# ypear/crdt

Measured on AMD Instinct MI355X. Metric: CRDT items merged/sec at 1/2/4/8 MI355X + % of HBM roofline, higher is better.
Workload: dtype u8/u32 (integer byte-stream + index work)

## Files before the change

### crdt_amd/csrc/yc_decode.hip

```cpp
#include <algorithm>
#include <cstdlib>

#include "yc_work.h"

namespace yc {

__device__ __forceinline__ uint64_t win8(const uint8_t* __restrict__ b, uint32_t p) {
  const uint32_t* d = (const uint32_t*)(b + (p & ~3u));
  return ((uint64_t)d[0] | ((uint64_t)d[1] << 32)) >> ((p & 3u) * 8);
}
__device__ __forceinline__ uint32_t win4(const uint8_t* __restrict__ b, uint32_t p) {
  const uint32_t* d = (const uint32_t*)(b + (p & ~3u));
  return __builtin_amdgcn_alignbyte(d[1], d[0], p & 3u);
}
struct RegWin {
  uint32_t r0, r1, r2, r3, r4, r5;
  uint32_t T;
  __device__ __forceinline__ static uint32_t sel(uint32_t m, uint32_t a1, uint32_t a0) { return (a1 & m) | (a0 & ~m); }
  __device__ __forceinline__ uint32_t word(uint32_t k) const {
    const uint32_t m0 = 0u - (k & 1u), m1 = 0u - ((k >> 1) & 1u), m2 = 0u - ((k >> 2) & 1u);
    const uint32_t a0 = sel(m0, r1, r0), a1 = sel(m0, r3, r2), a2 = sel(m0, r5, r4);
    return sel(m2, a2, sel(m1, a1, a0));
  }
  __device__ __forceinline__ uint32_t byte(uint32_t i) const { return (word(i >> 2) >> ((i & 3u) * 8)) & 0xFFu; }
// ... 2298 lines not shown
    uint32_t* out = k ? o1 : o0;
    uint32_t sum = 0;
    for (uint32_t i = a; i < e; ++i) sum += i < nwords ? (uint32_t)__popcll(bits[i]) : 0u;
    part[t] = sum;
    __syncthreads();
    for (uint32_t off = 1; off < COUNT_LANES; off <<= 1) {
      const uint32_t v = t >= off ? part[t - off] : 0u;
      __syncthreads();
      part[t] += v;
      __syncthreads();
    }
    uint32_t run = part[t] - sum;
    for (uint32_t i = a; i < e; ++i) { out[i] = run; run += i < nwords ? (uint32_t)__popcll(bits[i]) : 0u; }
    __syncthreads();
  }
}

void launch_struct_count(const Work& w, hipStream_t s) {
  const uint32_t nwords = (w.nbytes + 63) / 64;
  if (nwords + 1 <= COUNT_SMALL) {
    hipLaunchKernelGGL(k_count_small, dim3(1), dim3(COUNT_LANES), 0, s, w.final_bits, w.wcnt, w.sec_bits, w.wsec, nwords);
    return;
  }
  hipLaunchKernelGGL(k_popc, dim3(nwords / 256 + 1), dim3(256), 0, s, w.final_bits, w.scratch, nwords);
  scan_u32(w.tmp, w.tmp_bytes, w.scratch, w.wcnt, nwords + 1, s);
  hipLaunchKernelGGL(k_popc, dim3(nwords / 256 + 1), dim3(256), 0, s, w.sec_bits, w.scratch, nwords);
  scan_u32(w.tmp, w.tmp_bytes, w.scratch, w.wsec, nwords + 1, s);
}
void launch_struct_scatter(const Work& w, hipStream_t s) {
  const uint32_t nwords = (w.nbytes + 63) / 64;
  hipLaunchKernelGGL(k_scatter_pos, dim3(std::min<uint32_t>(nwords / 256 + 1, 4096)), dim3(256), 0, s, w.final_bits, w.wcnt, nwords, w.s_pos,
                     w.cap_structs, &w.ctr->err, w.nwin > 1 ? w.s_win : nullptr, w.win_shift);
}

void launch_section_clients(const Work& w, uint32_t nsections, hipStream_t s) {
  if (!nsections) return;
  hipLaunchKernelGGL(k_section_rank, dim3((nsections + 255) / 256), dim3(256), 0, s, w, nsections);
}

__device__ __forceinline__ uint32_t nth_lane(uint64_t x, uint32_t n) {
  for (uint32_t i = 0; i < n; ++i) x &= x - 1;
  return (uint32_t)__ffsll((long long)x) - 1;
}

__global__ __launch_bounds__(256) void k_ds_decode(Work w) {
  const uint32_t lane = threadIdx.x & 63;
// ... 812 lines not shown
__device__ __forceinline__ void struct_clock_at(const Work& w, uint32_t i, uint32_t nstructs, uint32_t states) {
  const uint32_t si = w.s_sec[i];
  const Section sec = w.sections[si];
  const uint64_t off = w.s_lenscan[i] - w.s_lenscan[sec.first_idx];
  const uint64_t clock = (uint64_t)sec.clock + off;
  const uint32_t len = w.s_len[i];
  const uint64_t endc = clock + len;
  if (endc > 0xFFFFFFFFull) { raise_err(&w.ctr->err, ERR_DECODE); return; }
  w.s_clock[i] = (uint32_t)clock;
  if (!states) return;
  const uint32_t ref = w.s_info[i] & 31u;
  if (ref == REF_SKIP) {
    atomicAdd(&w.ctr->items, (unsigned long long)len);
    return;
  }
  const bool last = i + 1 == nstructs || w.s_sec[i + 1] != si || (w.s_info[i + 1] & 31u) == REF_SKIP;
  if (last) atomicMax(&w.cl_state[w.s_cidx[i]], (uint32_t)endc);
}
__global__ void k_struct_clock(Work w, uint32_t nstructs, uint32_t states) {
  const uint32_t i = blockIdx.x * blockDim.x + threadIdx.x;
  if (i < nstructs) struct_clock_at(w, i, nstructs, states);
}

void launch_struct_decode(const Work& w, uint32_t nstructs, hipStream_t s) {
  if (!nstructs) return;
  hipLaunchKernelGGL(k_struct_decode, dim3((nstructs + 255) / 256), dim3(256), 0, s, w, nstructs);
  hipLaunchKernelGGL(k_struct_decode_deferred, dim3(std::min<uint32_t>(nstructs / 256 + 1, SD_DEFER_GRID)), dim3(256), 0, s, w);
}
void launch_struct_lenscan(const Work& w, uint32_t nstructs, hipStream_t s) {
  if (nstructs) scan_u32_to_u64(w.tmp, w.tmp_bytes, w.s_len, w.s_lenscan, nstructs + 1, s);
}

__device__ __forceinline__ void apply_caps_at(const Work& w, uint32_t c) {
  const uint32_t v = w.cl_vals[c];
  const uint32_t i = lower_bound_u32(w.cap_client, w.ncaps, v);
  const uint32_t cap = (i < w.ncaps && w.cap_client[i] == v) ? w.cap_clock[i] : 0u;
  if (ld_fresh(&w.cl_state[c]) > cap) w.cl_state[c] = cap;
}
__global__ void k_apply_caps(Work w) {
  const uint32_t c = blockIdx.x * blockDim.x + threadIdx.x;
  if (c < w.ctr->nclients) apply_caps_at(w, c);
}
__global__ void k_state_totals(Work w, uint32_t nstructs) {
  w.ctr->units = w.cl_base[w.ctr->nclients];
  w.ctr->in_len = w.s_lenscan[nstructs];
}
void launch_struct_clocks(const Work& w, uint32_t nstructs, hipStream_t s) {
  if (nstructs) hipLaunchKernelGGL(k_struct_clock, dim3((nstructs + 255) / 256), dim3(256), 0, s, w, nstructs, 0u);
}
void launch_states(const Work& w, uint32_t nstructs, uint32_t nsections, hipStream_t s) {
  if (nstructs) hipLaunchKernelGGL(k_struct_clock, dim3((nstructs + 255) / 256), dim3(256), 0, s, w, nstructs, 1u);
  if (w.capped && nsections) hipLaunchKernelGGL(k_apply_caps, dim3(nsections / 256 + 1), dim3(256), 0, s, w);
  scan_u32_to_u64(w.tmp, w.tmp_bytes, w.cl_state, w.cl_base, nsections + 1, s);
  hipLaunchKernelGGL(k_state_totals, dim3(1), dim3(1), 0, s, w, nstructs);
}

constexpr uint32_t DT_LANES = 256, DT_SMALL = 4096;
__global__ __launch_bounds__(DT_LANES) void k_decode_tail_small(Work w, uint32_t nstructs, uint32_t nsections) {
  __shared__ __attribute__((aligned(16))) uint32_t win[DT_LANES * SD_STRIDE];
  __shared__ uint64_t part[DT_LANES];
  const uint32_t t = threadIdx.x;
  if (nstructs == NONE) {
    if (w.ctr->err) return;
    nstructs = w.ctr->nstructs;
    nsections = w.ctr->nsections;
    if (nstructs > DT_SMALL || nsections + 1 > DT_LANES * 16) { if (t == 0) raise_err(&w.ctr->err, ERR_CAPACITY); return; }
  }
  if (w.dbg_bounds && (nstructs > w.cap_structs || nsections + 1 > w.cap_clients + 1)) {
    if (t == 0) bounds_fail(w.ctr, BOUNDS_DECODE_TAIL);
    return;
  }
  for (uint32_t i = t; i <= nsections; i += DT_LANES) { w.cl_start[i] = 0; w.cl_state[i] = 0; }
  for (uint32_t i = t; i < nstructs; i += DT_LANES) struct_decode_one<false>(w, i, win);
  __syncthreads();
  block_scan_u32_u64<DT_LANES>(w.s_len, w.s_lenscan, nstructs + 1, part);
  for (uint32_t i = t; i < nstructs; i += DT_LANES) struct_clock_at(w, i, nstructs, 1u);
  __syncthreads();
  const uint32_t nclients = w.ctr->nclients;
  if (w.capped) {
    for (uint32_t c = t; c < nclients; c += DT_LANES) apply_caps_at(w, c);
// ... 20 lines not shown
```

### crdt_amd/csrc/yc_engine.hip

```cpp
#include <cstddef>
#include <cstdio>
#include <cstring>
#include <string>
#include <vector>
#include <unordered_map>
#include <unordered_set>
#include <algorithm>
#include <memory>
#include <functional>

#include "yc_work.h"
#include "yc_host.h"
#include "yc_ingest.h"
#include "yc_comm.h"
#include "yc_sync.h"
#include "yc_json.h"
#include <thread>
#include <atomic>
#include "../../include/ycrdt.h"

using namespace yc;

namespace {

// ... 936 lines not shown
    uint32_t* fo = take<uint32_t>(V, B_FWCOFF, nu + 1, ok);
    if (ok) HIPCHK(hipMemcpyAsync(fo, b->fwc_off.data(), sizeof(uint32_t) * nu, hipMemcpyHostToDevice, e->stream));
    w.fwc_off = fo;
    if (!env_off("YCRDT_RTAB")) w.rtab = take<uint32_t>(V, B_RTAB, b->fwc_recs + 1, ok);
    if (w.rtab && !env_off("YCRDT_RANK_LAST")) w.rk = take<uint4>(V, B_RK, nu + 1, ok);
    const char* fw = getenv("YCRDT_FWC_WALK");
    w.fwc_walk = fw && atoi(fw) > 0 ? (uint32_t)atoi(fw) : 256u;
  }
  if (!ok) return fail(YCRDT_E_DEVICE, oom("decode workspace"));
  {
    size_t tb = prim_tmp_bytes(std::max<uint64_t>({B / 64 + 4, (uint64_t)nu + 2, (uint64_t)w.cap_sections + 2, 1024}),
                               (uint64_t)w.cap_sections + 2);
    w.tmp = take<uint8_t>(V, B_TMP, tb, ok);
    w.tmp_bytes = V[B_TMP].cap;
  }
  if (!ok) return fail(YCRDT_E_DEVICE, oom("scan scratch"));
  static_assert(sizeof(Counters) % 4 == 0, "counters are filled as words");
  fill_u32_multi({{(uint32_t*)w.ctr, sizeof(Counters) / 4, 0u},
                  {w.ufail, (uint64_t)nu + 1, 0u},
                  {w.usec_n, (uint64_t)nu + 1, 0u},
                  {(uint32_t*)w.final_bits, (uint64_t)nwords * 2, 0u},
                  {(uint32_t*)w.sec_bits, (uint64_t)nwords * 2, 0u}}, s);
  w.dbg_bounds = getenv("YCRDT_DEBUG_BOUNDS") && getenv("YCRDT_DEBUG_BOUNDS")[0] == '1' ? 1u : 0u;
  w.upre = b->pre_src >= 0 && !b->pre_check ? b->pre_u : NONE;
  if (w.upre != NONE) launch_predecoded(w, b->pre_u, b->pre, false, s);
  const bool dbg_yata = getenv("YCRDT_DEBUG_YATA") && getenv("YCRDT_DEBUG_YATA")[0] == '1';
  const bool dbg_dec = getenv("YCRDT_DEBUG_DECODE") && getenv("YCRDT_DEBUG_DECODE")[0] == '1';
  w.dbg = dbg_yata || dbg_dec ? take<unsigned long long>(V, B_DBG, 24, ok) : nullptr;
  if (w.dbg) HIPCHK(hipMemsetAsync(w.dbg, 0, 192, s));
  mark(e, "decode.direct");
  const bool split = sh && sh->comm && sh->nshards > 1 && !lazy;
  Work wd = w;
  if (split) {
    const int rc0 = split_decode_meta(e, b, sh, wd);
    if (rc0) return rc0;
  }
  const bool chunks = wd.ngroups || wd.nbig;
  if (chunks) {
    HIPCHK(hipEventRecord(e->side_fork, s));
    HIPCHK(hipStreamWaitEvent(e->side, e->side_fork, 0));
    launch_chunks(wd, e->side);
    HIPCHK(hipEventRecord(e->side_done, e->side));
  }
  launch_direct(wd, s);
  mark(e, "decode.chunk_wait");
  if (chunks) HIPCHK(hipStreamWaitEvent(s, e->side_done, 0));
// ... 25 lines not shown
  if (dbg_dec && w.dbg) {
    unsigned long long h[24];
    HIPCHK(hipMemcpy(h, w.dbg, sizeof(h), hipMemcpyDeviceToHost));
    fprintf(stderr, "[ycrdt decode] multi-section fast walk cycles: stage %llu walk %llu search %llu, walked structs %llu, sections vouched %llu\n",
            h[19], h[20], h[21], h[22], h[23]);
    fprintf(stderr, "[ycrdt decode] fastwalk: done %llu nsec %llu unsynced %llu | wave: done %llu unsettled %llu other %llu (chunk path: moved / jumped chunk entries) | k_spec exact parses %llu (%llu bytes) | multi-section left to k_walk, by reason 1-5: %llu %llu %llu %llu %llu (section %llu of %llu structs) | record mode: %llu sections evaluated by the walker, stopped at byte %llu of %llu\n",
            h[0], h[1], h[2], h[3], h[4], h[5], h[6], h[7], h[9], h[10], h[11], h[12], h[13], h[14], h[15], h[16], h[17], h[18]);
    HIPCHK(hipMemsetAsync(w.dbg, 0, 192, s));
  }
  if (rc == YCRDT_E_CAPACITY && !generous) return run_decode(e, b, lazy, D, true, sh);
  if (rc) return rc;
  const uint32_t nstructs = c.nstructs;
  const uint32_t nsections = c.nsections;
  w.cap_structs = nstructs + 64;
  w.cap_ds = c.ds_region + 64;
  w.cap_clients = nsections + 64;
  w.ds = lazy ? take<DsRange>(V, B_DS, w.cap_ds, ok) : nullptr;
  w.ds_tmp = take<DsRange>(V, B_DSTMP, w.cap_ds, ok);
  w.ds_len = nullptr;
  w.s_pos = take<uint32_t>(V, B_SPOS, w.cap_structs, ok);
  w.s_win = b->nwin > 1 ? take<uint8_t>(V, B_SWIN, w.cap_structs, ok) : nullptr;
  w.s_sec = take<uint32_t>(V, B_SSEC, w.cap_structs, ok);
  w.s_len = take<uint32_t>(V, B_SLEN, w.cap_structs + 1, ok);
  w.s_lenscan = take<uint64_t>(V, B_SLENSCAN, w.cap_structs + 1, ok);
  w.s_clock = take<uint32_t>(V, B_SCLOCK, w.cap_structs, ok);
  w.s_cidx = take<uint32_t>(V, B_SCIDX, w.cap_structs, ok);
  w.s_info = take<uint8_t>(V, B_SINFO, w.cap_structs, ok);
  w.s_ocidx = take<uint32_t>(V, B_SOC, w.cap_structs, ok);
  w.s_oclock = take<uint32_t>(V, B_SOK, w.cap_structs, ok);
  w.s_rcidx = take<uint32_t>(V, B_SRC, w.cap_structs, ok);
  w.s_rclock = take<uint32_t>(V, B_SRK, w.cap_structs, ok);
  w.s_pk = take<uint8_t>(V, B_SPK, w.cap_structs, ok);
  w.s_pa = take<uint32_t>(V, B_SPA, w.cap_structs, ok);
  w.s_pb = take<uint32_t>(V, B_SPB, w.cap_structs, ok);
  w.s_psub = take<uint32_t>(V, B_SPS, w.cap_structs, ok);
  w.s_psublen = take<uint32_t>(V, B_SPL, w.cap_structs, ok);
  w.s_cpos = take<uint32_t>(V, B_SCPOS, w.cap_structs, ok);
  w.s_cend = take<uint32_t>(V, B_SCEND, w.cap_structs, ok);
  w.s_celem = take<uint32_t>(V, B_SCELEM, w.cap_structs, ok);
  w.sd_defer = take<uint32_t>(V, B_SDDEFER, w.cap_structs, ok);
  w.cl_vals = take<uint32_t>(V, B_CLVALS, w.cap_clients + 1, ok);
  w.ch_key = nullptr;
  const uint32_t ch_slots = (uint32_t)next_pow2(std::max<uint64_t>(2ull * (nsections + 1), 64));
  uint64_t* ch_key = take<uint64_t>(V, B_CHKEY, ch_slots, ok);
  uint32_t* ch_val = take<uint32_t>(V, B_CHVAL, ch_slots, ok);
  w.cl_key = take<uint64_t>(V, B_CLKEY, w.cap_clients + 1, ok);
  w.cl_key2 = take<uint64_t>(V, B_CLKEY2, w.cap_clients + 1, ok);
// ... 52 lines not shown
    w.ch_key = ch_key;
    w.ch_val = ch_val;
    w.ch_mask = ch_slots - 1;
  } else if (nsections) {
    launch_client_table(w, nsections, s);
    fill_u32_multi({{(uint32_t*)ch_key, 2ull * ch_slots, 0xFFFFFFFFu}}, s);
    launch_client_hash(w, ch_key, ch_val, ch_slots - 1, s);
    w.ch_key = ch_key;
    w.ch_val = ch_val;
    w.ch_mask = ch_slots - 1;
  }
  mark(e, "decode.structs");
  if (quick) {
    launch_decode_tail_small(w, NONE, NONE, s);
    mark(e, "decode.clocks");
  } else if (!lazy && decode_tail_small(w, nstructs, nsections, s)) {
    mark(e, "decode.clocks");
  } else {
  launch_struct_decode(w, nstructs, s);
  mark(e, "decode.clocks");
  launch_struct_lenscan(w, nstructs, s);
  if (!lazy) {
    fill_u32_multi({{w.cl_start, (uint64_t)nsections + 1, 0u}, {w.cl_state, (uint64_t)nsections + 1, 0u}}, s);
    launch_states(w, nstructs, nsections, s);
  } else {
    HIPCHK(hipMemsetAsync(w.cl_start, 0, sizeof(uint32_t) * (nsections + 1), s));
    launch_struct_clocks(w, nstructs, s);
  }
  }
  HIPCHK(hipStreamWaitEvent(s, e->side_done, 0));
  rc = check(e, c, "struct decode");
  if (quick && rc == YCRDT_E_CAPACITY) return run_decode(e, b, lazy, D, true, sh);
  if (rc) return rc;
  const uint32_t nstructs_q = quick ? c.nstructs : nstructs, nsections_q = quick ? c.nsections : nsections;
  if (c.any_json) {
    w.jcap = std::max<uint32_t>(nstructs_q, 1);
    w.jlist = take<uint32_t>(V, B_JLIST, w.jcap, ok);
    if (!ok) return fail(YCRDT_E_DEVICE, oom("JSON list"));
    w.ntrusted = b->ntrusted;
    w.jskip_any = b->jpasses > 0 ? 1u : 0u;
    launch_json_structs(w, nstructs_q, s);
    rc = check(e, c, "JSON values");
    if (rc) return rc;
    if (c.njson) {
      bool restaged = false;
      if ((rc = json_rewrite(e, b, std::min(c.njson, w.jcap), sh, restaged))) return rc;
      if (restaged) return run_decode(e, b, lazy, D, generous, sh);
    }
  }
  D.noncanon = c.noncanon;
// ... 2664 lines not shown
```

### crdt_amd/csrc/yc_merge.hip

```cpp
#include <algorithm>
#include <cstdlib>

#include "yc_work.h"

namespace yc {



constexpr uint32_t LONG_UNITS = 32;
__device__ __forceinline__ uint64_t shfl64(uint64_t v, int l) {
  return ((uint64_t)(uint32_t)__shfl((uint32_t)(v >> 32), l) << 32) | (uint32_t)__shfl((uint32_t)v, l);
}
__device__ __forceinline__ void unit_owner(const Work& w, uint32_t nstructs, uint32_t s) {
  const uint32_t lane = threadIdx.x & 63;
  uint64_t gb = 0;
  uint32_t n = 0, fl = 0;
  if (s < nstructs) {
    const uint32_t ref = w.s_info[s] & 31u, cidx = w.s_cidx[s], clock = w.s_clock[s], len = w.s_len[s];
    const uint32_t st = w.cl_state[cidx];
    const uint64_t cb = w.cl_base[cidx];
    if (ref != REF_SKIP) {
      n = st > clock ? min(len, st - clock) : 0u;
      gb = cb + clock;
      fl = ref == REF_DELETED ? UF_DEL : (ref == REF_GC ? (UF_GC | UF_DEL) : 0u);
// ... 227 lines not shown
  if (blockIdx.x < nb) {
    const uint32_t s = blockIdx.x * blockDim.x + threadIdx.x;
    unit_owner(w, nstructs, s);
    unit_refs(w, nstructs, s);
  } else if (blockIdx.x < nb + nd) {
    unit_ds_apply(w, nclients, blockIdx.x - nb, BIG);
  } else if (BIG) {
    unit_ds_apply_big(w, nclients, blockIdx.x - nb - nd, nx);
  }
}
void launch_units_fill(const Work& w, uint64_t nunits, hipStream_t s) {
  fill_u32_multi({{w.u_owner, nunits, NONE}, {w.u_flags, nunits, 0u}}, s);
}
void launch_units(const Work& w, uint32_t nstructs, uint32_t nclients, uint32_t nds, uint64_t nunits, bool ds_big, hipStream_t s) {
  const uint32_t nb = (nstructs + 255) / 256, nd = nds && w.nupd ? (w.nupd + 3) / 4 : 0u;
  const uint32_t nx = nd && ds_big ? 256u : 0u;
  if (nb + nd) {
    if (nx) hipLaunchKernelGGL(k_units<true>, dim3(nb + nd + nx), dim3(256), 0, s, w, nstructs, nclients, nb, nd, nx);
    else hipLaunchKernelGGL(k_units<false>, dim3(nb + nd), dim3(256), 0, s, w, nstructs, nclients, nb, nd, 0u);
  }
  if (nx && w.ds_tails) hipLaunchKernelGGL(k_ds_tails, dim3(512), dim3(256), 0, s, w);
}

void launch_segments(const Work& w, uint32_t nclients, uint64_t nunits, hipStream_t s) {
  const uint32_t nwords = (uint32_t)((nunits + 63) / 64);
  if (nwords <= SEG_SMALL_WORDS) {
    hipLaunchKernelGGL(k_segments_small, dim3(1), dim3(SEG_LANES), 0, s, w, nunits);
    return;
  }
  hipLaunchKernelGGL(k_cuts, dim3(nwords / 4 + 1), dim3(256), 0, s, w, nunits);
  scan_u32(w.tmp, w.tmp_bytes, w.scratch, w.u_wpre, nwords + 1, s);
  hipLaunchKernelGGL(k_scatter_seg, dim3(nwords / 256 + 1), dim3(256), 0, s, w, nwords, nunits);
}

__device__ __forceinline__ uint64_t fnv_bytes(uint64_t h, const uint8_t* __restrict__ p, uint32_t n) {
  for (uint32_t i = 0; i < n; ++i) { h ^= p[i]; h *= 1099511628211ull; }
  return h;
}
__device__ __forceinline__ bool bytes_eq(const uint8_t* __restrict__ a, const uint8_t* __restrict__ b, uint32_t n) {
  for (uint32_t i = 0; i < n; ++i)
    if (a[i] != b[i]) return false;
  return true;
}
__device__ __forceinline__ bool same_list(const Work& w, uint32_t a, uint32_t b) {
  if (a == b) return true;
  const uint32_t pk = w.s_pk[a] & 3u;
  if (pk != (w.s_pk[b] & 3u)) return false;
  if (pk == 1) {
    const uint32_t n = w.s_pb[a];
    if (n != w.s_pb[b]) return false;
// ... 527 lines not shown
```

### crdt_amd/csrc/yc_prims.hip

```cpp
#include <algorithm>
#include <cstring>
#include <cstdlib>
#include <mutex>
#include <unordered_map>
#include <rocprim/rocprim.hpp>
#include "yc_work.h"

namespace yc {

struct SegMax64 {
  __host__ __device__ uint64_t operator()(uint64_t a, uint64_t b) const {
    return (a >> 32) == (b >> 32) ? (a > b ? a : b) : b;
  }
};

__global__ void k_fill_multi(FillBatch b) {
  const FillDesc d = b.d[blockIdx.y];
  for (uint64_t i = (uint64_t)blockIdx.x * blockDim.x + threadIdx.x; i < d.n; i += (uint64_t)gridDim.x * blockDim.x)
    d.p[i] = d.v;
}

void fill_u32_multi(std::initializer_list<FillDesc> fills, hipStream_t s) {
  FillBatch b{};
  uint64_t nmax = 0;
// ... 165 lines not shown
bool lb_launch(uint64_t tiles, uint32_t chains, hipStream_t s, LbChains& out) {
  std::lock_guard<std::mutex> g(lb_mu);
  LbState* st = lb_state(tiles * chains, s);
  if (!st) return false;
  out.state = st->state;
  out.stride = tiles;
  out.epoch = st->epoch;
  out.ord = st->state + st->tiles;
  out.ord_base = st->issued;
  st->issued += tiles;
  return true;
}

bool ordered_ids(uint64_t nblocks, hipStream_t s, OrderedIds& out) {
  std::lock_guard<std::mutex> g(lb_mu);
  LbState* st = lb_state(1, s);
  if (!st) return false;
  out.ctr = st->state + st->tiles;
  out.base = st->issued;
  st->issued += nblocks;
  return true;
}

void scan_u32(void* tmp, size_t tmpb, const uint32_t* in, uint32_t* out, uint64_t n, hipStream_t s) {
  if (!n) return;
  if (n <= SMALL_SCAN_MAX) {
    hipLaunchKernelGGL(k_scan_small<uint32_t>, dim3(1), dim3(SMALL_SCAN_LANES), 0, s, in, out, (uint32_t)n);
    return;
  }
  if (!getenv_flag("YCRDT_ROCPRIM_SCAN") && scan_lb<uint32_t>(in, out, n, s)) return;
  rocprim::exclusive_scan(tmp, tmpb, in, out, 0u, (size_t)n, rocprim::plus<uint32_t>(), s);
}

void scan_u32_to_u64(void* tmp, size_t tmpb, const uint32_t* in, uint64_t* out, uint64_t n, hipStream_t s) {
  if (!n) return;
  if (n <= SMALL_SCAN_MAX) {
    hipLaunchKernelGGL(k_scan_small<uint64_t>, dim3(1), dim3(SMALL_SCAN_LANES), 0, s, in, out, (uint32_t)n);
    return;
  }
  if (!getenv_flag("YCRDT_ROCPRIM_SCAN") && scan_lb<uint64_t>(in, out, n, s)) return;
  rocprim::exclusive_scan(tmp, tmpb, in, out, (uint64_t)0, (size_t)n, rocprim::plus<uint64_t>(), s);
}

void sort_u32(void* tmp, size_t tmpb, const uint32_t* in, uint32_t* out, uint64_t n, hipStream_t s) {
  if (!n) return;
  rocprim::radix_sort_keys(tmp, tmpb, in, out, (size_t)n, 0, 32, s);
// ... 35 lines not shown
```

### crdt_amd/csrc/yc_work.h

```cpp
#pragma once
#include <initializer_list>
#include "yc_common.h"
#include "yc_view.h"

namespace yc {

struct Counters {
  uint32_t err;
  uint32_t err_info;
  uint32_t nsections;
  uint32_t xchunks;
  uint32_t nds;
  uint32_t ndsclients;
  uint32_t nstructs;
  uint32_t nclients;
  uint32_t nunits_lo;
  uint32_t nunits_hi;
  uint32_t nsegs;
  uint32_t nout;
  uint32_t changed;
  uint32_t out_bytes;
  uint32_t sv_bytes;
  uint32_t nkeys;
  uint32_t nruns;
// ... 2 lines not shown
  uint32_t any_rorigin;
  uint32_t ds_big;
  uint32_t nsd_defer;
  uint32_t any_json;
  uint32_t narray_roots;
  uint32_t tgroups;
  uint32_t tbig;
  uint32_t ds_region;
  uint32_t nested;
  uint32_t nroots_sh[NSHARD];
  uint32_t nroots;
  uint32_t pad[12];
  uint32_t climb_open[40];
  uint32_t sync_changed[8];
  uint32_t noncanon;
  uint32_t lz_blocks;
  uint32_t njson;
  uint32_t ds_ntails;
  unsigned long long out_total;
  unsigned long long ds_base;
  unsigned long long items;
  unsigned long long units;
  unsigned long long in_len;
};

struct DsRange {
  uint32_t client;
  uint32_t clock;
  uint32_t len;
  uint32_t upd;
};

constexpr uint32_t WIN_SHIFT = 32;
__host__ __device__ inline uint64_t win_use(uint32_t shift) {
  return (1ull << shift) - (shift >= 28 ? (1ull << 20) : (1ull << 12));
}

struct Work {
  const uint8_t* bytes = nullptr;
  uint64_t nbytes = 0;
  uint32_t nwin = 1;
  uint32_t win_shift = WIN_SHIFT;
  const uint32_t* uwin = nullptr;
  const uint32_t* uoff = nullptr;
  const uint32_t* ulen = nullptr;
  const uint32_t* ugroup = nullptr;
  uint32_t nupd = 0;
  const uint32_t* udoc = nullptr;
  uint32_t ndocs = 1;
  const uint32_t* ulist = nullptr;
  uint32_t nbig = 0, nsmall = 0;
  uint32_t small_max = 0;
  uint32_t* fwsec = nullptr;
  uint4* fwc = nullptr;
  const uint32_t* fwc_off = nullptr;
  uint32_t* rtab = nullptr;
  uint4* rk = nullptr;
  uint32_t dbg_bounds = 0;
  uint32_t fwc_walk = 256;
  uint16_t* wlen = nullptr;
  uint32_t schunk = SCHUNK;
  uint32_t force_xtab = 0;
  uint32_t fwm_max = 0;
  uint32_t spec_hint = 2;
  uint32_t lazy = 0;
  unsigned long long* dbg = nullptr;
  const Group* groups = nullptr;
  uint32_t ngroups = 0;
  uint32_t cap_structs = 0, cap_sections = 0, cap_ds = 0, cap_dsclients = 0;
  uint64_t cap_units = 0;
  Counters* ctr = nullptr;
  uint64_t* spec_bits = nullptr;
  uint32_t* cexit = nullptr;
  uint32_t* sexit = nullptr;
  uint32_t* sent = nullptr;
  uint32_t* xtab = nullptr;
  uint32_t* tentry = nullptr;
  uint32_t* xlist = nullptr;
  uint32_t* ccnt = nullptr;
  uint32_t* coff = nullptr;
// ... 207 lines not shown
__device__ __forceinline__ uint32_t gidx() { return xcd_block() * blockDim.x + threadIdx.x; }

struct OrderedIds {
  unsigned long long* ctr = nullptr;
  unsigned long long base = 0;
};
bool ordered_ids(uint64_t nblocks, hipStream_t s, OrderedIds& out);
__device__ __forceinline__ uint32_t ordered_block_id(unsigned long long* ctr, unsigned long long base) {
  __shared__ uint32_t id;
  if (threadIdx.x == 0) id = (uint32_t)(atomicAdd(ctr, 1ull) - base);
  __syncthreads();
  return id;
}

constexpr uint64_t LB_VAL = (1ull << 40) - 1;
struct LbChains {
  unsigned long long* state = nullptr;
  uint64_t stride = 0;
  uint32_t epoch = 0;
  unsigned long long* ord = nullptr;
  unsigned long long ord_base = 0;
};
bool lb_launch(uint64_t tiles, uint32_t chains, hipStream_t s, LbChains& out);
__device__ __forceinline__ uint64_t lb_wave_lookback(unsigned long long* __restrict__ state, uint32_t tile, uint32_t epoch, uint64_t agg) {
  const uint32_t lane = threadIdx.x & 63;
  const unsigned long long ep = (unsigned long long)epoch << 42;
  if (tile == 0) {
    if (lane == 0) __hip_atomic_store(&state[0], ep | (2ull << 40) | (agg & LB_VAL), __ATOMIC_RELAXED, __HIP_MEMORY_SCOPE_AGENT);
    return 0;
  }
  if (lane == 0) __hip_atomic_store(&state[tile], ep | (1ull << 40) | (agg & LB_VAL), __ATOMIC_RELAXED, __HIP_MEMORY_SCOPE_AGENT);
  uint64_t pre = 0;
  for (int64_t j = (int64_t)tile - 1;; j -= 64) {
    const int64_t me = j - (int64_t)lane;
    uint32_t st = 2;
    uint64_t val = 0;
    if (me >= 0) {
      unsigned long long x;
      while (((x = __hip_atomic_load(&state[me], __ATOMIC_RELAXED, __HIP_MEMORY_SCOPE_AGENT)) >> 42) != epoch)
        __builtin_amdgcn_s_sleep(1);
      st = (uint32_t)(x >> 40) & 3u;
      val = x & LB_VAL;
    }
    const uint64_t done = __ballot(st == 2);
    const uint32_t stop = (uint32_t)__ffsll((long long)done) - 1;
    uint64_t part = lane <= stop ? val : 0ull;
    for (uint32_t off = 32; off > 0; off >>= 1) part += __shfl_xor(part, off);
    pre += part;
    if (done) break;
  }
  if (lane == 0) __hip_atomic_store(&state[tile], ep | (2ull << 40) | ((pre + agg) & LB_VAL), __ATOMIC_RELAXED, __HIP_MEMORY_SCOPE_AGENT);
  return pre;
}

__device__ __forceinline__ uint64_t client_hash(uint64_t k) {
  k ^= k >> 30; k *= 0xBF58476D1CE4E5B9ull;
  k ^= k >> 27; k *= 0x94D049BB133111EBull;
  return k ^ (k >> 31);
}
__device__ __forceinline__ uint32_t find_client(const Work& w, uint32_t nclients, uint32_t doc, uint32_t client) {
  if (w.ch_key) {
    const uint64_t key = w.udoc ? (((uint64_t)doc << 32) | client) : (uint64_t)client;
    for (uint32_t slot = (uint32_t)client_hash(key) & w.ch_mask;; slot = (slot + 1) & w.ch_mask) {
      const uint64_t k = w.ch_key[slot];
      if (k == key) return w.ch_val[slot];
      if (k == ~0ull) return NONE;
    }
  }
  if (!w.udoc) {
    const uint32_t i = lower_bound_u32(w.cl_vals, nclients, client);
    return (i < nclients && w.cl_vals[i] == client) ? i : NONE;
  }
  const uint64_t key = ((uint64_t)doc << 32) | client;
  uint32_t lo = 0, hi = nclients;
// ... 205 lines not shown
  uint32_t* order = nullptr;
  ViewSeg* segs = nullptr;
};
void launch_view(const Work& w, const ViewBufs& v, uint32_t nsegs, uint32_t nlists, uint32_t narr, hipStream_t s);

constexpr uint32_t UF_PRE = 6;
constexpr uint32_t UF_WALKED = 7;
struct PreMarks {
  uint64_t* fbits = nullptr;
  uint64_t* sbits = nullptr;
  Section* secs = nullptr;
  uint32_t* meta = nullptr;
  uint32_t nw = 0, cap_secs = 0;
};
void launch_state_marks(const Work& w, uint32_t nout, uint32_t nclients, const PreMarks& m, hipStream_t s);
void launch_predecoded(const Work& w, uint32_t u, const PreMarks& m, bool check, hipStream_t s);

void launch_chunks(const Work& w, hipStream_t s);
void launch_direct(const Work& w, hipStream_t s);
bool wave_decode(const Work& w);
void launch_client_hash(const Work& w, uint64_t* key, uint32_t* val, uint32_t mask, hipStream_t s);
bool sections_small(const Work& w, uint32_t nsections, uint64_t* key, uint32_t* val, uint32_t mask, hipStream_t s);
void launch_struct_count(const Work& w, hipStream_t s);
void launch_struct_scatter(const Work& w, hipStream_t s);
void launch_ds_bound(const Work& w, hipStream_t s);
bool count_ds_small(const Work& w, hipStream_t s);
void launch_ds_decode(const Work& w, hipStream_t s);
void launch_section_clients(const Work& w, uint32_t nsections, hipStream_t s);
void launch_client_table(Work& w, uint32_t nsections, hipStream_t s);
void launch_struct_decode(const Work& w, uint32_t nstructs, hipStream_t s);
void launch_struct_lenscan(const Work& w, uint32_t nstructs, hipStream_t s);
bool decode_tail_small(const Work& w, uint32_t nstructs, uint32_t nsections, hipStream_t s);
void launch_decode_tail_small(const Work& w, uint32_t nstructs, uint32_t nsections, hipStream_t s);
void launch_json_structs(const Work& w, uint32_t nstructs, hipStream_t s);
struct JItem {
  unsigned long long cpos;
  uint32_t clen;
  uint32_t len;
  uint32_t res;
  uint32_t pad;
};
void launch_json_canon(const Work& w, const uint32_t* list, uint32_t n, JItem* items, uint32_t* arena, uint32_t acap,
                       uint32_t lanes, const unsigned long long* offs, uint8_t* out, hipStream_t s);
void launch_states(const Work& w, uint32_t nstructs, uint32_t nsections, hipStream_t s);
void launch_struct_clocks(const Work& w, uint32_t nstructs, hipStream_t s);

void launch_units_fill(const Work& w, uint64_t nunits, hipStream_t s);
void launch_units(const Work& w, uint32_t nstructs, uint32_t nclients, uint32_t nds, uint64_t nunits, bool ds_big, hipStream_t s);
constexpr uint32_t DSA_WAVE = 4096;
void launch_segments(const Work& w, uint32_t nclients, uint64_t nunits, hipStream_t s);
void launch_segment_props_fill(const Work& w, uint32_t nsegs, hipStream_t s);
void launch_segment_props(const Work& w, uint32_t nsegs, uint32_t nclients, uint64_t nunits, hipStream_t s);
uint32_t run_key_resolution(const Work& w, uint32_t nsegs, hipStream_t s);
uint32_t run_descent(const Work& w, uint32_t nsegs, hipStream_t s, bool fold_overwrite);
void launch_mapx_flip(const Work& w, uint32_t nsegs, hipStream_t s);
void launch_mapx_fix(const Work& w, uint32_t nsegs, hipStream_t s);
bool merge_small_fits(uint64_t nsegs_bound);
void launch_merge_small(const Work& w, uint32_t nsegs, uint64_t nunits, hipStream_t s);
bool launch_merge_flags(const Work& w, uint32_t nsegs, hipStream_t s, bool fold_overwrite);
bool encode_runs_small(uint32_t nsegs);
void launch_merge_flags_only(const Work& w, uint32_t nsegs, hipStream_t s, bool fold_overwrite);
void launch_merge_tail(const Work& w, uint32_t nsegs, hipStream_t s);
void launch_key_shards(const Work& w, uint32_t nsegs, uint32_t nshards, uint32_t* key_shard, uint8_t* owner, hipStream_t s);
void launch_shard_mask(const Work& w, uint32_t nsegs, const uint8_t* owner, uint32_t shard, hipStream_t s);
void launch_shard_export(const Work& w, uint32_t nsegs, const uint8_t* owner, uint32_t shard, uint32_t* acc, hipStream_t s);
void launch_merge_final(const Work& w, uint32_t nsegs, hipStream_t s);
void run_dead_keys(const Work& w, uint32_t nsegs, hipStream_t s);
constexpr uint32_t DS_TAIL_MIN = 4096, DS_TAILS_CAP = 1u << 16;
// ... 49 lines not shown
```

Baseline: 3.864 billion.

## Fuse popcount scans, struct clocks, and segment cuts into single-pass look-back kernels

After: 4.036 billion, median of 6. +4.5%, better.

```diff
diff --git a/crdt_amd/csrc/yc_decode.hip b/crdt_amd/csrc/yc_decode.hip
--- a/crdt_amd/csrc/yc_decode.hip
+++ b/crdt_amd/csrc/yc_decode.hip
@@ -2344,6 +2344,7 @@
     hipLaunchKernelGGL(k_count_small, dim3(1), dim3(COUNT_LANES), 0, s, w.final_bits, w.wcnt, w.sec_bits, w.wsec, nwords);
     return;
   }
+  if (w.scan_fused && popc_scan2(w.final_bits, w.wcnt, w.sec_bits, w.wsec, nwords, s)) return;
   hipLaunchKernelGGL(k_popc, dim3(nwords / 256 + 1), dim3(256), 0, s, w.final_bits, w.scratch, nwords);
   scan_u32(w.tmp, w.tmp_bytes, w.scratch, w.wcnt, nwords + 1, s);
   hipLaunchKernelGGL(k_popc, dim3(nwords / 256 + 1), dim3(256), 0, s, w.sec_bits, w.scratch, nwords);
@@ -3202,13 +3203,134 @@
   if (i < nstructs) struct_clock_at(w, i, nstructs, states);
 }
 
+constexpr uint32_t SC_ITEMS = 16, SC_TILE = 256 * SC_ITEMS;
+constexpr uint64_t SC_SAT = 1ull << 33;
+__global__ __launch_bounds__(256) void k_struct_clock_lb(Work w, uint32_t nstructs, uint32_t states, uint32_t vec, LbChains lb) {
+  __shared__ uint64_t wsum[4], wlen[4];
+  __shared__ uint32_t whead[4];
+  __shared__ uint64_t tile_pre;
+  const uint32_t tile = ordered_block_id(lb.ord, lb.ord_base);
+  const uint32_t t = threadIdx.x, lane = t & 63, wv = t >> 6;
+  const uint64_t base = (uint64_t)tile * SC_TILE + (uint64_t)t * SC_ITEMS;
+  const bool full = vec && base + SC_ITEMS <= nstructs;
+  uint32_t sec[SC_ITEMS + 1], len[SC_ITEMS];
+  uint32_t info[SC_ITEMS + 1];
+  if (full) {
+#pragma unroll
+    for (uint32_t k = 0; k < SC_ITEMS / 4; ++k) {
+      const uint4 a = ((const uint4*)(w.s_sec + base))[k], b = ((const uint4*)(w.s_len + base))[k];
+      sec[4 * k] = a.x; sec[4 * k + 1] = a.y; sec[4 * k + 2] = a.z; sec[4 * k + 3] = a.w;
+      len[4 * k] = b.x; len[4 * k + 1] = b.y; len[4 * k + 2] = b.z; len[4 * k + 3] = b.w;
+    }
+    const uint4 q = *(const uint4*)(w.s_info + base);
+    const uint32_t qq[4] = {q.x, q.y, q.z, q.w};
+#pragma unroll
+    for (uint32_t k = 0; k < SC_ITEMS; ++k) info[k] = (qq[k >> 2] >> (8 * (k & 3))) & 0xFFu;
+  } else {
+#pragma unroll
+    for (uint32_t k = 0; k < SC_ITEMS; ++k) {
+      const bool in = base + k < nstructs;
+      sec[k] = in ? w.s_sec[base + k] : NONE;
+      len[k] = in ? w.s_len[base + k] : 0u;
+      info[k] = in ? (uint32_t)w.s_info[base + k] : 0u;
+    }
+  }
+  const bool nxt = base + SC_ITEMS < nstructs;
+  sec[SC_ITEMS] = nxt ? w.s_sec[base + SC_ITEMS] : NONE;
+  info[SC_ITEMS] = nxt ? (uint32_t)w.s_info[base + SC_ITEMS] : 0u;
+  const uint32_t psec = base > 0 && base <= nstructs ? w.s_sec[base - 1] : NONE;
+  uint64_t e[SC_ITEMS];
+  uint64_t run = 0, lsum = 0;
+  uint32_t heads = 0;
+#pragma unroll
+  for (uint32_t k = 0; k < SC_ITEMS; ++k) {
+    const bool in = base + k < nstructs;
+    const bool head = in && (base + k == 0 || sec[k] != (k ? sec[k - 1] : psec));
+    if (head) { run = w.sections[sec[k]].clock; heads |= 1u << k; }
+    run += len[k];
+    lsum += len[k];
+    e[k] = run;
+  }
+  uint64_t v = run;
+  uint32_t f = heads ? 1u : 0u;
+  for (uint32_t off = 1; off < 64; off <<= 1) {
+    const uint64_t pv = __shfl_up(v, off);
+    const uint32_t pf = __shfl_up(f, off);
+    if (lane >= off) { if (!f) v += pv; f |= pf; }
+  }
+  uint64_t ls = lsum;
+  for (uint32_t off = 32; off > 0; off >>= 1) ls += __shfl_xor(ls, off);
+  if (lane == 63) { wsum[wv] = v; whead[wv] = f; }
+  if (lane == 0) wlen[wv] = ls;
+  uint64_t cv = __shfl_up(v, 1);
+  uint32_t cf = __shfl_up(f, 1);
+  if (lane == 0) { cv = 0; cf = 0; }
+  __syncthreads();
+  uint64_t tv = 0;
+  uint32_t tf = 0;
+#pragma unroll
+  for (uint32_t x = 0; x < 4; ++x) {
+    if (x == wv) {
+      if (!cf) cv += tv;
+      cf |= tf;
+    }
+    if (whead[x]) { tv = wsum[x]; tf = 1u; } else tv += wsum[x];
+  }
+  if (wv == 0) {
+    const uint64_t pre = lb_wave_lookback(lb.state, tile, lb.epoch, tv, tf != 0, SC_SAT);
+    if (lane == 0) {
+      tile_pre = pre < SC_SAT ? pre : SC_SAT;
+      if (states) atomicAdd(&w.ctr->in_len_sh[tile & (NSHARD - 1)], (unsigned long long)(wlen[0] + wlen[1] + wlen[2] + wlen[3]));
+    }
+  }
+  __syncthreads();
+  const uint64_t carry = cf ? cv : cv + tile_pre;
+  const uint32_t first = heads ? (uint32_t)__ffs((int)heads) - 1 : SC_ITEMS;
+  uint32_t clk[SC_ITEMS];
+  uint32_t bad = 0;
+#pragma unroll
+  for (uint32_t k = 0; k < SC_ITEMS; ++k) {
+    const uint64_t endc = e[k] + (k < first ? carry : 0ull);
+    const bool in = base + k < nstructs;
+    const bool over = in && endc > 0xFFFFFFFFull;
+    bad |= (over ? 1u : 0u) << k;
+    clk[k] = (uint32_t)(endc - len[k]);
+    if (!in || over || !states) continue;
+    const uint32_t ref = info[k] & 31u;
+    if (ref == REF_SKIP) {
+      atomicAdd(&w.ctr->items, (unsigned long long)len[k]);
+      continue;
+    }
+    const bool last = base + k + 1 == nstructs || sec[k + 1] != sec[k] || (info[k + 1] & 31u) == REF_SKIP;
+    if (last) atomicMax(&w.cl_state[w.s_cidx[base + k]], (uint32_t)endc);
+  }
+  if (bad) raise_err(&w.ctr->err, ERR_DECODE);
+  if (full && !bad) {
+#pragma unroll
+    for (uint32_t k = 0; k < SC_ITEMS / 4; ++k)
+      ((uint4*)(w.s_clock + base))[k] = make_uint4(clk[4 * k], clk[4 * k + 1], clk[4 * k + 2], clk[4 * k + 3]);
+  } else {
+#pragma unroll
+    for (uint32_t k = 0; k < SC_ITEMS; ++k)
+      if (base + k < nstructs && !((bad >> k) & 1u)) w.s_clock[base + k] = clk[k];
+  }
+}
+static bool launch_struct_clock_lb(const Work& w, uint32_t nstructs, uint32_t states, hipStream_t s) {
+  const uint64_t tiles = ((uint64_t)nstructs + SC_TILE - 1) / SC_TILE;
+  LbChains lb;
+  if (!lb_launch(tiles, 1, s, lb)) return false;
+  const uint32_t vec = (((uintptr_t)w.s_sec | (uintptr_t)w.s_len | (uintptr_t)w.s_clock | (uintptr_t)w.s_info) & 15u) == 0;
+  hipLaunchKernelGGL(k_struct_clock_lb, dim3((uint32_t)tiles), dim3(256), 0, s, w, nstructs, states, vec, lb);
+  return true;
+}
+
 void launch_struct_decode(const Work& w, uint32_t nstructs, hipStream_t s) {
   if (!nstructs) return;
   hipLaunchKernelGGL(k_struct_decode, dim3((nstructs + 255) / 256), dim3(256), 0, s, w, nstructs);
   hipLaunchKernelGGL(k_struct_decode_deferred, dim3(std::min<uint32_t>(nstructs / 256 + 1, SD_DEFER_GRID)), dim3(256), 0, s, w);
 }
 void launch_struct_lenscan(const Work& w, uint32_t nstructs, hipStream_t s) {
-  if (nstructs) scan_u32_to_u64(w.tmp, w.tmp_bytes, w.s_len, w.s_lenscan, nstructs + 1, s);
+  if (nstructs && !clocks_fused(w, nstructs)) scan_u32_to_u64(w.tmp, w.tmp_bytes, w.s_len, w.s_lenscan, nstructs + 1, s);
 }
 
 __device__ __forceinline__ void apply_caps_at(const Work& w, uint32_t c) {
@@ -3221,21 +3343,29 @@
   const uint32_t c = blockIdx.x * blockDim.x + threadIdx.x;
   if (c < w.ctr->nclients) apply_caps_at(w, c);
 }
-__global__ void k_state_totals(Work w, uint32_t nstructs) {
+__global__ void k_state_totals(Work w, uint32_t nstructs, uint32_t fused) {
   w.ctr->units = w.cl_base[w.ctr->nclients];
-  w.ctr->in_len = w.s_lenscan[nstructs];
-}
-void launch_struct_clocks(const Work& w, uint32_t nstructs, hipStream_t s) {
+  if (!fused) { w.ctr->in_len = w.s_lenscan[nstructs]; return; }
+  unsigned long long n = 0;
+  for (uint32_t k = 0; k < NSHARD; ++k) n += w.ctr->in_len_sh[k];
+  w.ctr->in_len = n;
+}
+bool launch_struct_clocks(const Work& w, uint32_t nstructs, hipStream_t s) {
+  if (clocks_fused(w, nstructs)) return launch_struct_clock_lb(w, nstructs, 0u, s);
   if (nstructs) hipLaunchKernelGGL(k_struct_clock, dim3((nstructs + 255) / 256), dim3(256), 0, s, w, nstructs, 0u);
-}
-void launch_states(const Work& w, uint32_t nstructs, uint32_t nsections, hipStream_t s) {
-  if (nstructs) hipLaunchKernelGGL(k_struct_clock, dim3((nstructs + 255) / 256), dim3(256), 0, s, w, nstructs, 1u);
+  return true;
+}
+bool launch_states(const Work& w, uint32_t nstructs, uint32_t nsections, hipStream_t s) {
+  const bool fused = clocks_fused(w, nstructs);
+  if (fused) { if (!launch_struct_clock_lb(w, nstructs, 1u, s)) return false; }
+  else if (nstructs) hipLaunchKernelGGL(k_struct_clock, dim3((nstructs + 255) / 256), dim3(256), 0, s, w, nstructs, 1u);
   if (w.capped && nsections) hipLaunchKernelGGL(k_apply_caps, dim3(nsections / 256 + 1), dim3(256), 0, s, w);
   scan_u32_to_u64(w.tmp, w.tmp_bytes, w.cl_state, w.cl_base, nsections + 1, s);
-  hipLaunchKernelGGL(k_state_totals, dim3(1), dim3(1), 0, s, w, nstructs);
-}
-
-constexpr uint32_t DT_LANES = 256, DT_SMALL = 4096;
+  hipLaunchKernelGGL(k_state_totals, dim3(1), dim3(1), 0, s, w, nstructs, fused ? 1u : 0u);
+  return true;
+}
+
+constexpr uint32_t DT_LANES = 256;
 __global__ __launch_bounds__(DT_LANES) void k_decode_tail_small(Work w, uint32_t nstructs, uint32_t nsections) {
   __shared__ __attribute__((aligned(16))) uint32_t win[DT_LANES * SD_STRIDE];
   __shared__ uint64_t part[DT_LANES];
diff --git a/crdt_amd/csrc/yc_engine.hip b/crdt_amd/csrc/yc_engine.hip
--- a/crdt_amd/csrc/yc_engine.hip
+++ b/crdt_amd/csrc/yc_engine.hip
@@ -982,6 +982,7 @@
                   {(uint32_t*)w.final_bits, (uint64_t)nwords * 2, 0u},
                   {(uint32_t*)w.sec_bits, (uint64_t)nwords * 2, 0u}}, s);
   w.dbg_bounds = getenv("YCRDT_DEBUG_BOUNDS") && getenv("YCRDT_DEBUG_BOUNDS")[0] == '1' ? 1u : 0u;
+  w.scan_fused = env_off("YCRDT_SCAN_FUSED") ? 0u : 1u;
   w.upre = b->pre_src >= 0 && !b->pre_check ? b->pre_u : NONE;
   if (w.upre != NONE) launch_predecoded(w, b->pre_u, b->pre, false, s);
   const bool dbg_yata = getenv("YCRDT_DEBUG_YATA") && getenv("YCRDT_DEBUG_YATA")[0] == '1';
@@ -1053,7 +1054,7 @@
   w.s_win = b->nwin > 1 ? take<uint8_t>(V, B_SWIN, w.cap_structs, ok) : nullptr;
   w.s_sec = take<uint32_t>(V, B_SSEC, w.cap_structs, ok);
   w.s_len = take<uint32_t>(V, B_SLEN, w.cap_structs + 1, ok);
-  w.s_lenscan = take<uint64_t>(V, B_SLENSCAN, w.cap_structs + 1, ok);
+  w.s_lenscan = quick || !clocks_fused(w, nstructs) ? take<uint64_t>(V, B_SLENSCAN, w.cap_structs + 1, ok) : nullptr;
   w.s_clock = take<uint32_t>(V, B_SCLOCK, w.cap_structs, ok);
   w.s_cidx = take<uint32_t>(V, B_SCIDX, w.cap_structs, ok);
   w.s_info = take<uint8_t>(V, B_SINFO, w.cap_structs, ok);
@@ -1152,10 +1153,10 @@
   launch_struct_lenscan(w, nstructs, s);
   if (!lazy) {
     fill_u32_multi({{w.cl_start, (uint64_t)nsections + 1, 0u}, {w.cl_state, (uint64_t)nsections + 1, 0u}}, s);
-    launch_states(w, nstructs, nsections, s);
+    if (!launch_states(w, nstructs, nsections, s)) return fail(YCRDT_E_DEVICE, oom("look-back states"));
   } else {
     HIPCHK(hipMemsetAsync(w.cl_start, 0, sizeof(uint32_t) * (nsections + 1), s));
-    launch_struct_clocks(w, nstructs, s);
+    if (!launch_struct_clocks(w, nstructs, s)) return fail(YCRDT_E_DEVICE, oom("look-back states"));
   }
   }
   HIPCHK(hipStreamWaitEvent(s, e->side_done, 0));
diff --git a/crdt_amd/csrc/yc_merge.hip b/crdt_amd/csrc/yc_merge.hip
--- a/crdt_amd/csrc/yc_merge.hip
+++ b/crdt_amd/csrc/yc_merge.hip
@@ -273,10 +273,64 @@
   if (nx && w.ds_tails) hipLaunchKernelGGL(k_ds_tails, dim3(512), dim3(256), 0, s, w);
 }
 
+constexpr uint32_t SG_ITEMS = 16, SG_TILE = 256 * SG_ITEMS, SG_WORDS = SG_TILE / 64;
+__global__ __launch_bounds__(256) void k_segments_lb(Work w, uint32_t nwords, uint64_t nunits, LbChains lb) {
+  __shared__ uint64_t cw[SG_WORDS];
+  __shared__ uint32_t cp[SG_WORDS];
+  __shared__ uint32_t tile_pre;
+  const uint32_t tile = ordered_block_id(lb.ord, lb.ord_base);
+  const uint32_t lane = threadIdx.x & 63, wv = threadIdx.x >> 6;
+  const uint64_t g0 = (uint64_t)tile * SG_TILE;
+#pragma unroll 4
+  for (uint32_t k = 0; k < SG_ITEMS; ++k) {
+    const uint64_t word = __ballot(cut_at(w, g0 + k * 256 + threadIdx.x, nunits));
+    if (lane == 0) cw[k * 4 + wv] = word;
+  }
+  __syncthreads();
+  if (wv == 0) {
+    const uint64_t word = cw[lane];
+    const uint32_t c = (uint32_t)__popcll(word);
+    uint32_t inc = c;
+    for (uint32_t off = 1; off < 64; off <<= 1) {
+      const uint32_t y = __shfl_up(inc, off);
+      if (lane >= off) inc += y;
+    }
+    const uint32_t tot = __shfl(inc, 63);
+    const uint32_t pre = (uint32_t)lb_wave_lookback(lb.state, tile, lb.epoch, tot);
+    cp[lane] = inc - c;
+    if (lane == 0) tile_pre = pre;
+    const uint64_t wi = (uint64_t)tile * SG_WORDS + lane;
+    if (wi < nwords) {
+      w.u_cutbits[wi] = word;
+      w.u_wpre[wi] = pre + inc - c;
+    }
+    if (lane == 0 && g0 + SG_TILE >= nunits) {
+      const uint32_t nsegs = pre + tot;
+      w.u_wpre[nwords] = nsegs;
+      w.g_start[nsegs] = (uint32_t)nunits;
+      w.ctr->nsegs = nsegs;
+    }
+  }
+  __syncthreads();
+  const uint32_t base = tile_pre;
+  const uint64_t lt = (1ull << lane) - 1ull;
+#pragma unroll 4
+  for (uint32_t k = 0; k < SG_ITEMS; ++k) {
+    const uint64_t word = cw[k * 4 + wv];
+    if ((word >> lane) & 1ull) w.g_start[base + cp[k * 4 + wv] + (uint32_t)__popcll(word & lt)] = (uint32_t)(g0 + k * 256 + threadIdx.x);
+  }
+}
+
 void launch_segments(const Work& w, uint32_t nclients, uint64_t nunits, hipStream_t s) {
   const uint32_t nwords = (uint32_t)((nunits + 63) / 64);
   if (nwords <= SEG_SMALL_WORDS) {
     hipLaunchKernelGGL(k_segments_small, dim3(1), dim3(SEG_LANES), 0, s, w, nunits);
+    return;
+  }
+  const uint64_t tiles = (nunits + SG_TILE - 1) / SG_TILE;
+  LbChains lb;
+  if (w.scan_fused && lb_launch(tiles, 1, s, lb)) {
+    hipLaunchKernelGGL(k_segments_lb, dim3((uint32_t)tiles), dim3(256), 0, s, w, nwords, nunits, lb);
     return;
   }
   hipLaunchKernelGGL(k_cuts, dim3(nwords / 4 + 1), dim3(256), 0, s, w, nunits);
diff --git a/crdt_amd/csrc/yc_prims.hip b/crdt_amd/csrc/yc_prims.hip
--- a/crdt_amd/csrc/yc_prims.hip
+++ b/crdt_amd/csrc/yc_prims.hip
@@ -211,6 +211,78 @@
   return true;
 }
 
+__global__ __launch_bounds__(LB_LANES) void k_popc_scan2(const uint64_t* __restrict__ b0, uint32_t* __restrict__ o0,
+                                                        const uint64_t* __restrict__ b1, uint32_t* __restrict__ o1, uint32_t nwords,
+                                                        uint32_t vec, LbChains lb) {
+  __shared__ uint32_t wtot[2][LB_LANES / 64];
+  __shared__ uint32_t tile_pre[2];
+  const uint32_t tile = ordered_block_id(lb.ord, lb.ord_base);
+  const uint32_t t = threadIdx.x, lane = t & 63, wv = t >> 6;
+  const uint64_t base = (uint64_t)tile * LB_TILE + (uint64_t)t * LB_ITEMS;
+  const bool full = vec && base + LB_ITEMS <= nwords;
+  uint32_t v[2][LB_ITEMS], sum[2], inc[2];
+#pragma unroll
+  for (uint32_t c = 0; c < 2; ++c) {
+    const uint64_t* __restrict__ bits = c ? b1 : b0;
+    if (full) {
+#pragma unroll
+      for (uint32_t k = 0; k < LB_ITEMS / 2; ++k) {
+        const ulonglong2 q = ((const ulonglong2*)(bits + base))[k];
+        v[c][2 * k] = (uint32_t)__popcll(q.x);
+        v[c][2 * k + 1] = (uint32_t)__popcll(q.y);
+      }
+    } else {
+#pragma unroll
+      for (uint32_t k = 0; k < LB_ITEMS; ++k) v[c][k] = base + k < nwords ? (uint32_t)__popcll(bits[base + k]) : 0u;
+    }
+    sum[c] = 0;
+#pragma unroll
+    for (uint32_t k = 0; k < LB_ITEMS; ++k) sum[c] += v[c][k];
+    inc[c] = sum[c];
+    for (uint32_t off = 1; off < 64; off <<= 1) {
+      const uint32_t y = __shfl_up(inc[c], off);
+      if (lane >= off) inc[c] += y;
+    }
+    if (lane == 63) wtot[c][wv] = inc[c];
+  }
+  __syncthreads();
+  if (wv < 2) {
+    uint32_t agg = 0;
+#pragma unroll
+    for (uint32_t k = 0; k < LB_LANES / 64; ++k) agg += wtot[wv][k];
+    const uint32_t pre = (uint32_t)lb_wave_lookback(lb.state + (wv ? lb.stride : 0), tile, lb.epoch, agg);
+    if (lane == 0) tile_pre[wv] = pre;
+  }
+  __syncthreads();
+#pragma unroll
+  for (uint32_t c = 0; c < 2; ++c) {
+    uint32_t* __restrict__ out = c ? o1 : o0;
+    uint32_t run = tile_pre[c] + inc[c] - sum[c];
+#pragma unroll
+    for (uint32_t k = 0; k < LB_LANES / 64; ++k) run += k < wv ? wtot[c][k] : 0u;
+    uint32_t o[LB_ITEMS];
+#pragma unroll
+    for (uint32_t k = 0; k < LB_ITEMS; ++k) { o[k] = run; run += v[c][k]; }
+    if (vec && base + LB_ITEMS <= (uint64_t)nwords + 1) {
+#pragma unroll
+      for (uint32_t k = 0; k < LB_ITEMS / 4; ++k)
+        ((uint4*)(out + base))[k] = make_uint4(o[4 * k], o[4 * k + 1], o[4 * k + 2], o[4 * k + 3]);
+    } else {
+#pragma unroll
+      for (uint32_t k = 0; k < LB_ITEMS; ++k)
+        if (base + k <= nwords) out[base + k] = o[k];
+    }
+  }
+}
+bool popc_scan2(const uint64_t* b0, uint32_t* o0, const uint64_t* b1, uint32_t* o1, uint32_t nwords, hipStream_t s) {
+  const uint64_t tiles = ((uint64_t)nwords + 1 + LB_TILE - 1) / LB_TILE;
+  LbChains lb;
+  if (!lb_launch(tiles, 2, s, lb)) return false;
+  const uint32_t vec = (((uintptr_t)b0 | (uintptr_t)b1 | (uintptr_t)o0 | (uintptr_t)o1) & 15u) == 0;
+  hipLaunchKernelGGL(k_popc_scan2, dim3((uint32_t)tiles), dim3(LB_LANES), 0, s, b0, o0, b1, o1, nwords, vec, lb);
+  return true;
+}
+
 void scan_u32(void* tmp, size_t tmpb, const uint32_t* in, uint32_t* out, uint64_t n, hipStream_t s) {
   if (!n) return;
   if (n <= SMALL_SCAN_MAX) {
diff --git a/crdt_amd/csrc/yc_work.h b/crdt_amd/csrc/yc_work.h
--- a/crdt_amd/csrc/yc_work.h
+++ b/crdt_amd/csrc/yc_work.h
@@ -48,6 +48,7 @@
   unsigned long long items;
   unsigned long long units;
   unsigned long long in_len;
+  unsigned long long in_len_sh[NSHARD];
 };
 
 struct DsRange {
@@ -82,6 +83,7 @@
   const uint32_t* fwc_off = nullptr;
   uint32_t* rtab = nullptr;
   uint4* rk = nullptr;
+  uint32_t scan_fused = 1;
   uint32_t dbg_bounds = 0;
   uint32_t fwc_walk = 256;
   uint16_t* wlen = nullptr;
@@ -335,14 +337,16 @@
   unsigned long long ord_base = 0;
 };
 bool lb_launch(uint64_t tiles, uint32_t chains, hipStream_t s, LbChains& out);
-__device__ __forceinline__ uint64_t lb_wave_lookback(unsigned long long* __restrict__ state, uint32_t tile, uint32_t epoch, uint64_t agg) {
+__device__ __forceinline__ uint64_t lb_wave_lookback(unsigned long long* __restrict__ state, uint32_t tile, uint32_t epoch, uint64_t agg,
+                                                     bool closed = false, uint64_t sat = 0) {
   const uint32_t lane = threadIdx.x & 63;
   const unsigned long long ep = (unsigned long long)epoch << 42;
+  auto pack = [&](uint64_t v) -> unsigned long long { return sat ? (v < sat ? v : sat) : (v & LB_VAL); };
   if (tile == 0) {
-    if (lane == 0) __hip_atomic_store(&state[0], ep | (2ull << 40) | (agg & LB_VAL), __ATOMIC_RELAXED, __HIP_MEMORY_SCOPE_AGENT);
+    if (lane == 0) __hip_atomic_store(&state[0], ep | (2ull << 40) | pack(agg), __ATOMIC_RELAXED, __HIP_MEMORY_SCOPE_AGENT);
     return 0;
   }
-  if (lane == 0) __hip_atomic_store(&state[tile], ep | (1ull << 40) | (agg & LB_VAL), __ATOMIC_RELAXED, __HIP_MEMORY_SCOPE_AGENT);
+  if (lane == 0) __hip_atomic_store(&state[tile], ep | ((closed ? 2ull : 1ull) << 40) | pack(agg), __ATOMIC_RELAXED, __HIP_MEMORY_SCOPE_AGENT);
   uint64_t pre = 0;
   for (int64_t j = (int64_t)tile - 1;; j -= 64) {
     const int64_t me = j - (int64_t)lane;
@@ -362,7 +366,7 @@
     pre += part;
     if (done) break;
   }
-  if (lane == 0) __hip_atomic_store(&state[tile], ep | (2ull << 40) | ((pre + agg) & LB_VAL), __ATOMIC_RELAXED, __HIP_MEMORY_SCOPE_AGENT);
+  if (!closed && lane == 0) __hip_atomic_store(&state[tile], ep | (2ull << 40) | pack(pre + agg), __ATOMIC_RELAXED, __HIP_MEMORY_SCOPE_AGENT);
   return pre;
 }
 
@@ -614,6 +618,7 @@
 void launch_client_hash(const Work& w, uint64_t* key, uint32_t* val, uint32_t mask, hipStream_t s);
 bool sections_small(const Work& w, uint32_t nsections, uint64_t* key, uint32_t* val, uint32_t mask, hipStream_t s);
 void launch_struct_count(const Work& w, hipStream_t s);
+bool popc_scan2(const uint64_t* b0, uint32_t* o0, const uint64_t* b1, uint32_t* o1, uint32_t nwords, hipStream_t s);
 void launch_struct_scatter(const Work& w, hipStream_t s);
 void launch_ds_bound(const Work& w, hipStream_t s);
 bool count_ds_small(const Work& w, hipStream_t s);
@@ -622,6 +627,8 @@
 void launch_client_table(Work& w, uint32_t nsections, hipStream_t s);
 void launch_struct_decode(const Work& w, uint32_t nstructs, hipStream_t s);
 void launch_struct_lenscan(const Work& w, uint32_t nstructs, hipStream_t s);
+constexpr uint32_t DT_SMALL = 4096;
+inline bool clocks_fused(const Work& w, uint32_t nstructs) { return w.scan_fused && nstructs > DT_SMALL; }
 bool decode_tail_small(const Work& w, uint32_t nstructs, uint32_t nsections, hipStream_t s);
 void launch_decode_tail_small(const Work& w, uint32_t nstructs, uint32_t nsections, hipStream_t s);
 void launch_json_structs(const Work& w, uint32_t nstructs, hipStream_t s);
@@ -634,8 +641,8 @@
 };
 void launch_json_canon(const Work& w, const uint32_t* list, uint32_t n, JItem* items, uint32_t* arena, uint32_t acap,
                        uint32_t lanes, const unsigned long long* offs, uint8_t* out, hipStream_t s);
-void launch_states(const Work& w, uint32_t nstructs, uint32_t nsections, hipStream_t s);
-void launch_struct_clocks(const Work& w, uint32_t nstructs, hipStream_t s);
+bool launch_states(const Work& w, uint32_t nstructs, uint32_t nsections, hipStream_t s);
+bool launch_struct_clocks(const Work& w, uint32_t nstructs, hipStream_t s);
 
 void launch_units_fill(const Work& w, uint64_t nunits, hipStream_t s);
 void launch_units(const Work& w, uint32_t nstructs, uint32_t nclients, uint32_t nds, uint64_t nunits, bool ds_big, hipStream_t s);
```
